# nv-dvl/nerfmatch

Hardware: AMD Instinct MI355X
Metric: rays*samples/sec (higher is better)
Workload: dtype fp16x3 (fp16 MFMA on hi/lo-split fp32 operands, three products per fp32 product, fp32 accumulate; fp32 everywhere else)

## Files before the change

### nerfmatch_amd/csrc/nerf_points_bf16.hip

```cpp
#include "nerf_split_chain.h"

namespace {
using namespace nmbf;
using nmsample::HALF_PI_F32, nmsample::frustum, nmsample::ray_consts, nmsample::lift_var, nmsample::ipe_exact, nmsample::view_row_value;

struct PointsArgs {
  const char* blob;
  const float* xi;
  const float* xd;
  const float* g4;
  float* out4;
  float* g_xi0;
  float* g_xi5;
  float* g_xd;
  u32x4* gates;
  int n, ntiles;
  const float* rays;
  const float* z;
  const float* app_row;
  int S, Sa;
  float* feats;
  const float* tap_w;
  const float* tap_g;
  int tap;
// ... 116 lines not shown
          if (ob < 2) gv0 |= bit; else gv1 |= bit;
          pr = NM_FMA(hv, wr4[e], pr);
          pg = NM_FMA(hv, wg4[e], pg);
          pb = NM_FMA(hv, wb4[e], pb);
        }
      }
    cx.gptr[8 * 256] = u32x4{gv0, gv1, 0u, 0u};
    pr = (pr + nm_shfl_xor32(pr)) + sm_small[OFF_MISC + 1];
    pg = (pg + nm_shfl_xor32(pg)) + sm_small[OFF_MISC + 2];
    pb = (pb + nm_shfl_xor32(pb)) + sm_small[OFF_MISC + 3];
    const float sigma_raw = (cx.sig_part + nm_shfl_xor32(cx.sig_part)) + sm_small[OFF_MISC];
    if (hh == 0 && sample < a.n) *reinterpret_cast<f32x4*>(a.out4 + (size_t)sample * 4) = f32x4{pr, pg, pb, sigma_raw};
  }
}

template <bool GATED>
struct UnitWorkB {
  Ctx& cx;
  Unit& out;
  int u;
  u32x4 gw;
  float v8[8];
  float f0, f1;
  __device__ __forceinline__ void prefetch() {}
  __device__ __forceinline__ void operator()(int j) {
    const int ob = u >> 1, m = u & 1;
    if (j < 4) {
      float a0 = cx.hv[ob * 16 + 8 * m + j], a1 = cx.hv[ob * 16 + 8 * m + 4 + j];
      if constexpr (GATED) {
        const unsigned w = gw[u >> 2];
        const int base = 8 * (u & 3);
        const int e0 = j, e1 = 4 + j;
        const int b0 = base + ((e0 & 1) ? 4 + (e0 >> 1) : (e0 >> 1)), b1 = base + ((e1 & 1) ? 4 + (e1 >> 1) : (e1 >> 1));
        a0 = __int_as_float(__float_as_int(a0) & __builtin_amdgcn_sbfe((int)w, b0, 1));
        a1 = __int_as_float(__float_as_int(a1) & __builtin_amdgcn_sbfe((int)w, b1, 1));
      }
      v8[j] = a0; v8[4 + j] = a1;
      pin(v8[j]); pin(v8[4 + j]);
    } else if (!(j & 1)) {
      const int p = (j - 4) >> 1;
      unsigned hp = pack_bf16(v8[2 * p], v8[2 * p + 1]);
      f0 = __uint_as_float(hp << 16);
      f1 = __uint_as_float(hp & 0xffff0000u);
      pin(hp); pin(f0); pin(f1);
      out.h[p] = hp;
    } else {
      const int p = (j - 5) >> 1;
      float r0 = v8[2 * p] - f0, r1 = v8[2 * p + 1] - f1;
      pin(r0); pin(r1);
      unsigned lp = pack_bf16(r0, r1);
      pin(lp);
      out.l[p] = lp;
    }
  }
};
template <bool GATED>
__device__ __forceinline__ UnitWorkB<GATED> unit_work_b(int u, Ctx& cx, Unit& out, const u32x4& gw) {
  return UnitWorkB<GATED>{cx, out, u, gw, {}, 0.f, 0.f};
}
template <bool GATED>
__device__ __forceinline__ void make_unit0_b(Ctx& cx, const u32x4& gw) {
  UnitWorkB<GATED> w = unit_work_b<GATED>(0, cx, cx.xn, gw);
#pragma unroll
  for (int j = 0; j < 12; ++j) w(j);
}
template <int NOB, int NKS, bool GATED>
__device__ __forceinline__ void bwd_product(f32x16 (&acc)[NOB], Ctx& cx, const u32x4& gw) {
#pragma unroll
  for (int ks = 0; ks < NKS; ks += 2) {
    {
      const Unit xc = cx.xn;
      const bf16x8 xh = __builtin_bit_cast(bf16x8, xc.h), xl = __builtin_bit_cast(bf16x8, xc.l);
      if constexpr (NOB == 8) {
        if (ks == 0) slot_step8<0, true, true>(acc, cx, xh, xl, unit_work_b<GATED>(ks + 1, cx, cx.xn, gw));
        else slot_step8<0, false, true>(acc, cx, xh, xl, unit_work_b<GATED>(ks + 1, cx, cx.xn, gw));
      } else {
        if (ks == 0) slot_step4<0, true, true>(acc, cx, xh, xl, unit_work_b<GATED>(ks + 1, cx, cx.xn, gw));
        else slot_step4<0, false, true>(acc, cx, xh, xl, unit_work_b<GATED>(ks + 1, cx, cx.xn, gw));
      }
    }
    {
      const Unit xc = cx.xn;
      const bf16x8 xh = __builtin_bit_cast(bf16x8, xc.h), xl = __builtin_bit_cast(bf16x8, xc.l);
      if constexpr (NOB == 8) {
        if (ks + 2 < NKS) slot_step8<0, false, false>(acc, cx, xh, xl, unit_work_b<GATED>(ks + 2, cx, cx.xn, gw));
        else slot_step8<0, false, false>(acc, cx, xh, xl, NoWork{});
      } else {
// ... 169 lines not shown
```

### nerfmatch_amd/csrc/nerf_split_chain.h

```cpp
#pragma once
#include "nerf_bf16_common.h"

namespace nmbf {

template <int P> constexpr bool is_bf16() { return P == 0 || P == 4; }
template <int P> constexpr bool has_gates() { return P == 4; }
typedef _Float16 f16x8 __attribute__((ext_vector_type(8)));
typedef _Float16 f16x2 __attribute__((ext_vector_type(2)));
template <int P>
__device__ __forceinline__ f32x16 mfma_p(const bf16x8& a, const bf16x8& b, const f32x16& c) {
  if constexpr (is_bf16<P>()) return MFMA_BF16(a, b, c);
  else return __builtin_amdgcn_mfma_f32_32x32x16_f16(__builtin_bit_cast(f16x8, a), __builtin_bit_cast(f16x8, b), c, 0, 0, 0);
}
template <int P> constexpr bool is_split() { return P != 1; }
template <int P> constexpr int slot_bytes() { return is_split<P>() ? SLOT_BYTES : SLOT_BYTES / 2; }
template <int P> constexpr int slot_floats() { return slot_bytes<P>() / 4; }
template <int P> constexpr int ring_slots() { return is_split<P>() ? NRING : 2 * NRING; }
template <int P> constexpr int ring_ahead() { return is_split<P>() ? 4 : 6; }
constexpr float F16_MAX = 65504.0f;
__device__ __forceinline__ void split8_f16(const float (&v)[8], bf16x8& hi, bf16x8& lo) {
  f16x8 h8, l8;
#pragma unroll
  for (int i = 0; i < 8; ++i) {
    const float c = __builtin_amdgcn_fmed3f(v[i], -F16_MAX, F16_MAX);
// ... 92 lines not shown
      d.l[o] = __builtin_bit_cast(bf16x8, s4[((4 * p + o) * 2 + 1) * 64]);
    } else {
      d.h[o] = __builtin_bit_cast(bf16x8, s4[(4 * p + o) * 64]);
    }
  }
}

struct Ctx {
  const char* blob_slots;
  float* ring;
  const float* sm_small;
  f32x4* tapw;
  bool tap_pref;
  bool rgb;
  float* tap_ring;
  float* tap_ipe;
  int nslots, wave, lane, hi;
  int tap;
  int g;
  unsigned dma_voff;
  unsigned dma_lds;
  OpHalf opA;
  OpHalf opB;
  Unit xn;
  float sig_part;
  float sc;
  float vmax;
  unsigned* rng;
  u32x4* gptr;
  unsigned gbits[4];
  float hv[128];
};

template <int P>
__device__ __forceinline__ void ring_request(const Ctx& cx, int g, int j) {
  const int slot = g + 2 + (j >> 2);
  const char* base = cx.blob_slots + (size_t)slot * slot_bytes<P>();
  const unsigned lds = cx.dma_lds + (unsigned)(slot & (ring_slots<P>() - 1)) * slot_bytes<P>();
  unsigned m0_saved;
#define NM_DMA_PIECE(OFS)                                                                                                        \
  asm volatile("s_mov_b32 %0, m0\n\ts_mov_b32 m0, %1\n\tglobal_load_lds_dwordx4 %2, %3 offset:" #OFS "\n\ts_mov_b32 m0, %0" \
               : "=&s"(m0_saved) : "s"(lds), "v"(cx.dma_voff), "s"(base) : "memory")
  switch (j & 3) {
    case 0: NM_DMA_PIECE(0); break;
    case 1: NM_DMA_PIECE(1024); break;
    case 2: NM_DMA_PIECE(2048); break;
// ... 7 lines not shown
  for (int g0 = 0; g0 < (is_split<P>() ? 2 : ring_ahead<P>()); ++g0) dma_slot<P>(blob_slots, g0, ring, wave, lane);
}
template <int P>
__device__ __forceinline__ void ring_open_wait(Ctx& cx) {
  cx.dma_voff = (unsigned)(cx.wave * (slot_bytes<P>() / 4) + cx.lane * 16);
  const float* q = cx.ring + cx.wave * (slot_floats<P>() / 4);
  cx.dma_lds = (unsigned)__builtin_amdgcn_readfirstlane((int)(unsigned)(size_t)(const __attribute__((address_space(3))) float*)q);
  NM_WAIT_VMCNT(0);
  __builtin_amdgcn_s_barrier();
}

__device__ __forceinline__ unsigned gate_byte(const u32x4& h) {
  const unsigned w0 = h[0], w1 = h[1], w2 = h[2], w3 = h[3];
  unsigned m0, m1, m2, m3;
  const unsigned one = 0x00010001u;
  asm("v_pk_min_u16 %0, %1, %2" : "=v"(m0) : "v"(w0), "v"(one));
  asm("v_pk_min_u16 %0, %1, %2" : "=v"(m1) : "v"(w1), "v"(one));
  asm("v_pk_min_u16 %0, %1, %2" : "=v"(m2) : "v"(w2), "v"(one));
  asm("v_pk_min_u16 %0, %1, %2" : "=v"(m3) : "v"(w3), "v"(one));
  const unsigned t = m0 | (m1 << 1) | (m2 << 2) | (m3 << 3);
  return (t & 0xfu) | ((t >> 12) & 0xf0u);
}

template <int P>
struct UnitWork {
  Ctx& cx;
  Unit& out;
  int u, lo;
  float floor_v;
  f32x4 b0, b1;
  float sc;
  float v8[8];
  float f0, f1;
  unsigned hpk;
  __device__ __forceinline__ void prefetch() {
    const int ob = u >> 1, m = u & 1;
    const float* bl = cx.sm_small + OFF_BIAS + lo * 256 + ob * 32 + 16 * m + 4 * cx.hi;
    b0 = *reinterpret_cast<const f32x4*>(bl); b1 = *reinterpret_cast<const f32x4*>(bl + 8);
  }
  __device__ __forceinline__ void operator()(int j) {
    const int ob = u >> 1, m = u & 1;
    if (j < 4) {
      if constexpr (is_bf16<P>()) {
        v8[j] = __builtin_fmaxf(cx.hv[ob * 16 + 8 * m + j] + b0[j], floor_v);
        v8[4 + j] = __builtin_fmaxf(cx.hv[ob * 16 + 8 * m + 4 + j] + b1[j], floor_v);
      } else if constexpr (P == 1) {
        v8[j] = __builtin_amdgcn_fmed3f(cx.hv[ob * 16 + 8 * m + j] + b0[j], floor_v, F16_MAX);
        v8[4 + j] = __builtin_amdgcn_fmed3f(cx.hv[ob * 16 + 8 * m + 4 + j] + b1[j], floor_v, F16_MAX);
      } else {
        v8[j] = __builtin_amdgcn_fmed3f(__builtin_fmaf(cx.hv[ob * 16 + 8 * m + j], sc, b0[j]), floor_v, F16_MAX);
        v8[4 + j] = __builtin_amdgcn_fmed3f(__builtin_fmaf(cx.hv[ob * 16 + 8 * m + 4 + j], sc, b1[j]), floor_v, F16_MAX);
        asm("v_max3_f32 %0, |%1|, |%2|, %0" : "+v"(cx.vmax) : "v"(v8[j]), "v"(v8[4 + j]));
      }
      pin(v8[j]); pin(v8[4 + j]);
    } else if constexpr (P == 1) {
      if (j < 8) {
        unsigned hp = pack_f16(v8[2 * (j - 4)], v8[2 * (j - 4) + 1]);
        pin(hp);
        out.h[j - 4] = hp;
      }
    } else if (!(j & 1)) {
      const int p = (j - 4) >> 1;
      unsigned hp;
      if constexpr (is_bf16<P>()) {
        hp = pack_bf16(v8[2 * p], v8[2 * p + 1]);
        f0 = __uint_as_float(hp << 16);
        f1 = __uint_as_float(hp & 0xffff0000u);
      } else {
        hp = pack_f16(v8[2 * p], v8[2 * p + 1]);
        hpk = hp;
      }
      pin(hp);
      if constexpr (is_bf16<P>()) { pin(f0); pin(f1); }
      out.h[p] = hp;
    } else {
      const int p = (j - 5) >> 1;
      float r0, r1;
      if constexpr (is_bf16<P>()) {
        r0 = v8[2 * p] - f0; r1 = v8[2 * p + 1] - f1;
      } else {
        asm("v_fma_mix_f32 %0, %1, -1.0, %2 op_sel:[0,0,0] op_sel_hi:[1,0,0]" : "=v"(r0) : "v"(hpk), "v"(v8[2 * p]));
        asm("v_fma_mix_f32 %0, %1, -1.0, %2 op_sel:[1,0,0] op_sel_hi:[1,0,0]" : "=v"(r1) : "v"(hpk), "v"(v8[2 * p + 1]));
      }
      pin(r0); pin(r1);
      unsigned lp = is_bf16<P>() ? pack_bf16(r0, r1) : pack_f16(r0, r1);
      pin(lp);
      out.l[p] = lp;
      if constexpr (has_gates<P>()) {
        if (j == 11) {
          const unsigned t = gate_byte(out.h);
          cx.gbits[u >> 2] |= t << (8 * (u & 3));
        }
      }
    }
  }
};
template <int P>
__device__ __forceinline__ void fold_range(Ctx& cx, int slot) {
  if constexpr (P == 2) {
    const unsigned addr = (unsigned)(size_t)(const __attribute__((address_space(3))) unsigned*)(cx.rng + slot * 256);
    asm volatile("ds_max_u32 %0, %1" :: "v"(addr), "v"(__float_as_uint(cx.vmax)) : "memory");
    cx.vmax = 0.f;
  }
}
struct NoWork {
  __device__ __forceinline__ void prefetch() {}
  __device__ __forceinline__ void operator()(int) {}
};
template <int P>
struct AccTake {
  const f32x16 (&acc)[8];
  Ctx& cx;
  __device__ __forceinline__ void prefetch() {}
  __device__ __forceinline__ void operator()(int j) {
    constexpr int per = is_split<P>() ? 6 : 8;
#pragma unroll
    for (int k = 0; k < per; ++k) {
      const int i = per * j + k;
      if (i < 64) cx.hv[i] = acc_read(acc[i >> 4][i & 15]);
    }
  }
};
template <int P>
__device__ __forceinline__ UnitWork<P> unit_work(int u, int lo, Ctx& cx, Unit& out) {
  return UnitWork<P>{cx, out, u, lo, lo < 8 ? 0.f : (!is_bf16<P>() ? -F16_MAX : -__builtin_inff()), {}, {}, cx.sc, {}, 0.f, 0.f, 0u};
}

template <int P>
__device__ __forceinline__ void finish_layer(const f32x16 (&acc)[8], int l, Ctx& cx) {
#pragma unroll
  for (int ob = 4; ob < 8; ++ob)
#pragma unroll
    for (int r = 0; r < 16; ++r) cx.hv[ob * 16 + r] = acc_read(acc[ob][r]);
  if constexpr (P == 2)
    cx.sc = __builtin_bit_cast(float, __builtin_amdgcn_readfirstlane(__builtin_bit_cast(int, cx.sm_small[OFF_SCALE + l])));
  UnitWork<P> w = unit_work<P>(0, l, cx, cx.xn);
  w.prefetch();
#pragma unroll
  for (int j = 0; j < 12; ++j) w(j);
}

__device__ __forceinline__ void alpha_head(Ctx& cx) {
  const float* bl = cx.sm_small + OFF_BIAS + 7 * 256 + 4 * cx.hi;
  const float* wa = cx.sm_small + OFF_WALPHA + 4 * cx.hi;
  const float s7 = cx.sm_small[OFF_SCALE + 7];
  float p0 = 0.f, p1 = 0.f, p2 = 0.f, p3 = 0.f;
#pragma unroll
  for (int ob = 0; ob < 8; ++ob)
#pragma unroll
    for (int q = 0; q < 4; ++q) {
      const f32x4 b = *reinterpret_cast<const f32x4*>(bl + ob * 32 + 8 * q);
      const f32x4 w4v = *reinterpret_cast<const f32x4*>(wa + ob * 32 + 8 * q);
      p0 = NM_FMA(__builtin_fmaxf(__builtin_fmaf(cx.hv[ob * 16 + 4 * q + 0], s7, b[0]), 0.f), w4v[0], p0);
      p1 = NM_FMA(__builtin_fmaxf(__builtin_fmaf(cx.hv[ob * 16 + 4 * q + 1], s7, b[1]), 0.f), w4v[1], p1);
      p2 = NM_FMA(__builtin_fmaxf(__builtin_fmaf(cx.hv[ob * 16 + 4 * q + 2], s7, b[2]), 0.f), w4v[2], p2);
      p3 = NM_FMA(__builtin_fmaxf(__builtin_fmaf(cx.hv[ob * 16 + 4 * q + 3], s7, b[3]), 0.f), w4v[3], p3);
    }
  cx.sig_part = (p0 + p1) + (p2 + p3);
}

__device__ __forceinline__ void dump_tap(int lo, Ctx& cx) {
  const float* bl = cx.sm_small + OFF_BIAS + lo * 256 + 4 * cx.hi;
  const float sl = cx.sm_small[OFF_SCALE + lo];
  auto* tp = (__attribute__((address_space(1))) f32x4*)cx.tapw;
#pragma unroll
  for (int ob = 0; ob < 8; ++ob) {
    f32x4 v[4];
#pragma unroll
    for (int q = 0; q < 4; ++q) {
      const f32x4 b = *reinterpret_cast<const f32x4*>(bl + ob * 32 + 8 * q);
#pragma unroll
      for (int e = 0; e < 4; ++e) v[q][e] = __builtin_fmaxf(__builtin_fmaf(cx.hv[ob * 16 + 4 * q + e], sl, b[e]), 0.f);
    }
#pragma unroll
    for (int q = 0; q < 4; ++q) tp[q * 64] = v[q];
    tp += 256;
    pin(tp);
  }
}

template <int P, bool FIRST, int NOB>
__device__ __forceinline__ void mfma_head(f32x16 (&acc)[NOB], int p, const OpHalf& a, const bf16x8& xh) {
  const f32x16 zero = {0.f, 0.f, 0.f, 0.f, 0.f, 0.f, 0.f, 0.f, 0.f, 0.f, 0.f, 0.f, 0.f, 0.f, 0.f, 0.f};
#pragma unroll
  for (int o = 0; o < 4; ++o) acc[4 * p + o] = mfma_p<P>(a.h[o], xh, FIRST ? zero : acc[4 * p + o]);
}
template <int P, int NOB>
__device__ __forceinline__ void mfma_tail(f32x16 (&acc)[NOB], int p, const OpHalf& a, const bf16x8& xh, const bf16x8& xl) {
#pragma unroll
  for (int o = 0; o < 4; ++o) acc[4 * p + o] = mfma_p<P>(a.h[o], xl, acc[4 * p + o]);
#pragma unroll
  for (int o = 0; o < 4; ++o) acc[4 * p + o] = mfma_p<P>(a.l[o], xh, acc[4 * p + o]);
}

__device__ __forceinline__ bf16x8 load_op1(const float* slot, int lane, int blk) {
  return __builtin_bit_cast(bf16x8, (reinterpret_cast<const u32x4*>(slot) + lane)[blk * 64]);
}
#define NM_SB __builtin_amdgcn_sched_barrier(0)
template <bool FIRST, bool ACQ, class Work>
__device__ __forceinline__ void slot_step8_one(f32x16 (&acc)[8], Ctx& cx, const bf16x8& x, Work work) {
  const f32x16 zero = {0.f, 0.f, 0.f, 0.f, 0.f, 0.f, 0.f, 0.f, 0.f, 0.f, 0.f, 0.f, 0.f, 0.f, 0.f, 0.f};
  const int g = cx.g;
  const OpHalf A = cx.opA, B = cx.opB;
  const float* nxt = ring_slot<1>(cx.ring, g + 1);
  acc[0] = mfma_p<1>(A.h[0], x, FIRST ? zero : acc[0]); NM_SB;
  if constexpr (ACQ) ring_acquire_pair(cx.blob_slots, g, cx.ring, cx.wave, cx.lane);
  NM_SB;
  acc[1] = mfma_p<1>(A.h[1], x, FIRST ? zero : acc[1]); NM_SB;
  cx.opA.h[0] = load_op1(nxt, cx.lane, 0); cx.opA.h[1] = load_op1(nxt, cx.lane, 1); work.prefetch(); NM_SB;
  acc[2] = mfma_p<1>(A.h[2], x, FIRST ? zero : acc[2]); NM_SB;
  cx.opA.h[2] = load_op1(nxt, cx.lane, 2); cx.opA.h[3] = load_op1(nxt, cx.lane, 3); NM_SB;
  acc[3] = mfma_p<1>(A.h[3], x, FIRST ? zero : acc[3]); NM_SB;
  cx.opB.h[0] = load_op1(nxt, cx.lane, 4); cx.opB.h[1] = load_op1(nxt, cx.lane, 5); NM_SB;
  acc[4] = mfma_p<1>(B.h[0], x, FIRST ? zero : acc[4]); NM_SB;
  cx.opB.h[2] = load_op1(nxt, cx.lane, 6); cx.opB.h[3] = load_op1(nxt, cx.lane, 7); NM_SB;
  acc[5] = mfma_p<1>(B.h[1], x, FIRST ? zero : acc[5]); NM_SB;
  work(0); work(1); NM_SB;
  acc[6] = mfma_p<1>(B.h[2], x, FIRST ? zero : acc[6]); NM_SB;
  work(2); work(3); work(4); NM_SB;
  acc[7] = mfma_p<1>(B.h[3], x, FIRST ? zero : acc[7]); NM_SB;
  work(5); work(6); work(7); NM_SB;
  cx.g = g + 1;
}

template <int P, bool FIRST, bool EVEN, class Work>
__device__ __forceinline__ void slot_step8(f32x16 (&acc)[8], Ctx& cx, const bf16x8& xh, const bf16x8& xl, Work work) {
  if constexpr (P == 1) {
    slot_step8_one<FIRST, EVEN>(acc, cx, xh, work);
    return;
  }
  const f32x16 zero = {0.f, 0.f, 0.f, 0.f, 0.f, 0.f, 0.f, 0.f, 0.f, 0.f, 0.f, 0.f, 0.f, 0.f, 0.f, 0.f};
  const int g = cx.g;
  OpHalf B;
  mfma_head<P, FIRST, 8>(acc, 0, cx.opA, xh);
  __builtin_amdgcn_sched_barrier(0);
  load_half<P>(B, cx.ring + (g & (NRING - 1)) * SLOT_FLOATS, cx.lane, 1);
  work.prefetch();
  __builtin_amdgcn_sched_barrier(0);
  if constexpr (EVEN) {
#pragma unroll
    for (int o = 0; o < 8; ++o) {
      acc[o & 3] = mfma_p<P>(o < 4 ? cx.opA.h[o & 3] : cx.opA.l[o & 3], o < 4 ? xl : xh, acc[o & 3]);
      ring_request<P>(cx, g, o);
      __builtin_amdgcn_sched_barrier(0);
    }
  } else {
    mfma_tail<P, 8>(acc, 0, cx.opA, xh, xl);
    __builtin_amdgcn_sched_barrier(0);
    ring_acquire_two();
    __builtin_amdgcn_sched_barrier(0);
  }
#pragma unroll
  for (int o = 0; o < 4; ++o) {
    acc[4 + o] = mfma_p<P>(B.h[o], xh, FIRST ? zero : acc[4 + o]);
    __builtin_amdgcn_sched_barrier(0);
    work(o);
    __builtin_amdgcn_sched_barrier(0);
  }
  load_half<P>(cx.opA, cx.ring + ((g + 1) & (NRING - 1)) * SLOT_FLOATS, cx.lane, 0);
  __builtin_amdgcn_sched_barrier(0);
#pragma unroll
  for (int o = 0; o < 4; ++o) {
    acc[4 + o] = mfma_p<P>(B.h[o], xl, acc[4 + o]);
    __builtin_amdgcn_sched_barrier(0);
    work(4 + o);
    __builtin_amdgcn_sched_barrier(0);
  }
#pragma unroll
  for (int o = 0; o < 4; ++o) {
    acc[4 + o] = mfma_p<P>(B.l[o], xh, acc[4 + o]);
    __builtin_amdgcn_sched_barrier(0);
    work(8 + o);
    __builtin_amdgcn_sched_barrier(0);
  }
  cx.g = g + 1;
}

template <bool FIRST, bool ACQ, class Work>
__device__ __forceinline__ void slot_step4_one(f32x16 (&acc)[4], Ctx& cx, const bf16x8& x, Work work) {
  const f32x16 zero = {0.f, 0.f, 0.f, 0.f, 0.f, 0.f, 0.f, 0.f, 0.f, 0.f, 0.f, 0.f, 0.f, 0.f, 0.f, 0.f};
  const int g = cx.g;
  const OpHalf C = cx.opA;
  const float* nxt = ring_slot<1>(cx.ring, g + 1);
  acc[0] = mfma_p<1>(C.h[0], x, FIRST ? zero : acc[0]); NM_SB;
  if constexpr (ACQ) ring_acquire_pair(cx.blob_slots, g, cx.ring, cx.wave, cx.lane);
  NM_SB;
  acc[1] = mfma_p<1>(C.h[1], x, FIRST ? zero : acc[1]); NM_SB;
#pragma unroll
  for (int o = 0; o < 4; ++o) cx.opA.h[o] = load_op1(nxt, cx.lane, o);
  work.prefetch(); NM_SB;
  acc[2] = mfma_p<1>(C.h[2], x, FIRST ? zero : acc[2]); NM_SB;
  work(0); work(1); work(2); work(3); NM_SB;
  acc[3] = mfma_p<1>(C.h[3], x, FIRST ? zero : acc[3]); NM_SB;
  work(4); work(5); work(6); work(7); NM_SB;
  cx.g = g + 1;
}

template <int P, bool FIRST, bool EVEN, class Work>
__device__ __forceinline__ void slot_step4(f32x16 (&acc)[4], Ctx& cx, const bf16x8& xh, const bf16x8& xl, Work work) {
  if constexpr (P == 1) {
    slot_step4_one<FIRST, EVEN>(acc, cx, xh, work);
    return;
  }
  const f32x16 zero = {0.f, 0.f, 0.f, 0.f, 0.f, 0.f, 0.f, 0.f, 0.f, 0.f, 0.f, 0.f, 0.f, 0.f, 0.f, 0.f};
  const int g = cx.g;
  const OpHalf C = cx.opA;
  work.prefetch();
  if constexpr (!EVEN) ring_acquire_two();
#pragma unroll
  for (int o = 0; o < 4; ++o) {
    acc[o] = mfma_p<P>(C.h[o], xh, FIRST ? zero : acc[o]);
    __builtin_amdgcn_sched_barrier(0);
    work(o);
    __builtin_amdgcn_sched_barrier(0);
  }
  load_half<P>(cx.opA, cx.ring + ((g + 1) & (NRING - 1)) * SLOT_FLOATS, cx.lane, 0);
  __builtin_amdgcn_sched_barrier(0);
#pragma unroll
  for (int o = 0; o < 4; ++o) {
    acc[o] = mfma_p<P>(C.h[o], xl, acc[o]);
    __builtin_amdgcn_sched_barrier(0);
    if constexpr (EVEN) ring_request<P>(cx, g, o);
    work(4 + o);
    __builtin_amdgcn_sched_barrier(0);
  }
#pragma unroll
  for (int o = 0; o < 4; ++o) {
    acc[o] = mfma_p<P>(C.l[o], xh, acc[o]);
    __builtin_amdgcn_sched_barrier(0);
    if constexpr (EVEN) ring_request<P>(cx, g, 4 + o);
    work(8 + o);
    __builtin_amdgcn_sched_barrier(0);
  }
  cx.g = g + 1;
}

template <int P, bool FIRST, bool EVEN, class W0, class W1>
__device__ __forceinline__ void slot_step4x2(f32x16 (&av)[4], Ctx& cx, const bf16x8& x0h, const bf16x8& x0l, Unit& u1, W0 w0, W1 w1) {
  const f32x16 zero = {0.f, 0.f, 0.f, 0.f, 0.f, 0.f, 0.f, 0.f, 0.f, 0.f, 0.f, 0.f, 0.f, 0.f, 0.f, 0.f};
  const int g = cx.g;
  const OpHalf A = cx.opA;
  OpHalf B;
  w0.prefetch();
#pragma unroll
  for (int o = 0; o < 4; ++o) {
    av[o] = mfma_p<P>(A.h[o], x0h, FIRST ? zero : av[o]);
    __builtin_amdgcn_sched_barrier(0);
    w0(o);
    __builtin_amdgcn_sched_barrier(0);
  }
  load_half<P>(B, cx.ring + (g & (NRING - 1)) * SLOT_FLOATS, cx.lane, 1);
  __builtin_amdgcn_sched_barrier(0);
#pragma unroll
  for (int o = 0; o < 4; ++o) {
    av[o] = mfma_p<P>(A.h[o], x0l, av[o]);
    __builtin_amdgcn_sched_barrier(0);
    if constexpr (EVEN) ring_request<P>(cx, g, o);
    w0(4 + o);
    __builtin_amdgcn_sched_barrier(0);
  }
#pragma unroll
  for (int o = 0; o < 4; ++o) {
    av[o] = mfma_p<P>(A.l[o], x0h, av[o]);
    __builtin_amdgcn_sched_barrier(0);
    if constexpr (EVEN) ring_request<P>(cx, g, 4 + o);
    w0(8 + o);
    __builtin_amdgcn_sched_barrier(0);
  }
  if constexpr (!EVEN) {
    ring_acquire_two();
    __builtin_amdgcn_sched_barrier(0);
  }
  const bf16x8 x1h = __builtin_bit_cast(bf16x8, u1.h), x1l = __builtin_bit_cast(bf16x8, u1.l);
  w1.prefetch();
#pragma unroll
  for (int o = 0; o < 4; ++o) {
    av[o] = mfma_p<P>(B.h[o], x1h, av[o]);
    __builtin_amdgcn_sched_barrier(0);
    w1(o);
    __builtin_amdgcn_sched_barrier(0);
  }
  load_half<P>(cx.opA, cx.ring + ((g + 1) & (NRING - 1)) * SLOT_FLOATS, cx.lane, 0);
  __builtin_amdgcn_sched_barrier(0);
#pragma unroll
  for (int o = 0; o < 4; ++o) {
    av[o] = mfma_p<P>(B.h[o], x1l, av[o]);
    __builtin_amdgcn_sched_barrier(0);
    w1(4 + o);
    __builtin_amdgcn_sched_barrier(0);
  }
#pragma unroll
  for (int o = 0; o < 4; ++o) {
    av[o] = mfma_p<P>(B.l[o], x1h, av[o]);
    __builtin_amdgcn_sched_barrier(0);
    w1(8 + o);
    __builtin_amdgcn_sched_barrier(0);
  }
  cx.g = g + 1;
}

template <int P>
__device__ __forceinline__ void views_hidden(f32x16 (&av)[4], Ctx& cx) {
  if constexpr (is_split<P>()) {
#pragma unroll
    for (int sl = 0; sl < HS / 2; ++sl) {
      const Unit x0 = cx.xn;
      Unit u1;
      const bf16x8 x0h = __builtin_bit_cast(bf16x8, x0.h), x0l = __builtin_bit_cast(bf16x8, x0.l);
      if (sl == 0) slot_step4x2<P, true, true>(av, cx, x0h, x0l, u1, unit_work<P>(1, 7, cx, u1), unit_work<P>(2, 7, cx, cx.xn));
      else if (sl + 1 == HS / 2) slot_step4x2<P, false, false>(av, cx, x0h, x0l, u1, unit_work<P>(2 * sl + 1, 7, cx, u1), NoWork{});
      else if (sl & 1) slot_step4x2<P, false, false>(av, cx, x0h, x0l, u1, unit_work<P>(2 * sl + 1, 7, cx, u1), unit_work<P>(2 * sl + 2, 7, cx, cx.xn));
      else slot_step4x2<P, false, true>(av, cx, x0h, x0l, u1, unit_work<P>(2 * sl + 1, 7, cx, u1), unit_work<P>(2 * sl + 2, 7, cx, cx.xn));
    }
  } else {
#pragma unroll
    for (int ks = 0; ks < HS; ks += 2) {
      {
        const Unit xc = cx.xn;
// ... 3 lines not shown
      {
        const Unit xc = cx.xn;
        if (ks + 2 < HS) slot_step4<P, false, false>(av, cx, __builtin_bit_cast(bf16x8, xc.h), __builtin_bit_cast(bf16x8, xc.l), unit_work<P>(ks + 2, 7, cx, cx.xn));
        else slot_step4<P, false, false>(av, cx, __builtin_bit_cast(bf16x8, xc.h), __builtin_bit_cast(bf16x8, xc.l), NoWork{});
      }
    }
  }
}
template <int P>
__device__ __forceinline__ void views_extras(f32x16 (&av)[4], Ctx& cx, const bf16x8 (&eh)[VS], const bf16x8 (&el)[VS], bool no_app) {
  if constexpr (is_split<P>()) {
    Unit u1;
    u1.h = __builtin_bit_cast(u32x4, eh[1]); u1.l = __builtin_bit_cast(u32x4, el[1]);
    slot_step4x2<P, false, true>(av, cx, eh[0], el[0], u1, NoWork{}, NoWork{});
    if (!no_app) slot_step4<P, false, false>(av, cx, eh[2], el[2], NoWork{});
  } else {
    slot_step4<P, false, true>(av, cx, eh[0], el[0], NoWork{});
    slot_step4<P, false, false>(av, cx, eh[1], el[1], NoWork{});
    if (!no_app) slot_step4<P, false, true>(av, cx, eh[2], el[2], NoWork{});
  }
}

template <int P, bool FIRST>
__device__ __forceinline__ void ipe_steps(f32x16 (&acc)[8], Ctx& cx, const float* ipe_src) {
  auto operand = [&](int m, bf16x8& ph, bf16x8& pl) {
    ph = __builtin_bit_cast(bf16x8, *reinterpret_cast<const u32x4*>(ipe_src + (is_split<P>() ? (m * 2 + 0) : m) * 256));
    pl = ph;
    if constexpr (is_split<P>()) pl = __builtin_bit_cast(bf16x8, *reinterpret_cast<const u32x4*>(ipe_src + (m * 2 + 1) * 256));
  };
#pragma unroll
  for (int m = 0; m < XS; m += 2) {
    bf16x8 ph, pl;
    operand(m, ph, pl);
    if (m == 0) slot_step8<P, FIRST, true>(acc, cx, ph, pl, NoWork{});
    else slot_step8<P, false, true>(acc, cx, ph, pl, NoWork{});
    operand(m + 1, ph, pl);
    if (m + 2 == XS) slot_step8<P, false, false>(acc, cx, ph, pl, AccTake<P>{acc, cx});
    else slot_step8<P, false, false>(acc, cx, ph, pl, NoWork{});
  }
}

struct Tap7Workspace {
  static constexpr bool on = false;
  __device__ __forceinline__ void fn(Ctx&) const {}
};
template <class F>
struct Tap7InRegisters {
  bool on;
  F fn;
};

template <int P, class Tap7 = Tap7Workspace>
__device__ __forceinline__ void layer_pass(f32x16 (&acc)[8], int l, Ctx& cx, const float* ipe_src, const Tap7& tap7 = Tap7()) {
  if (l - 1 == cx.tap) dump_tap(l - 1, cx);
#pragma unroll
  for (int ks = 0; ks < HS; ks += 2) {
    {
      const Unit xc = cx.xn;
      if (ks == 0) slot_step8<P, true, true>(acc, cx, __builtin_bit_cast(bf16x8, xc.h), __builtin_bit_cast(bf16x8, xc.l), unit_work<P>(ks + 1, l - 1, cx, cx.xn));
      else slot_step8<P, false, true>(acc, cx, __builtin_bit_cast(bf16x8, xc.h), __builtin_bit_cast(bf16x8, xc.l), unit_work<P>(ks + 1, l - 1, cx, cx.xn));
    }
    {
      const Unit xc = cx.xn;
      if (ks + 2 < HS) slot_step8<P, false, false>(acc, cx, __builtin_bit_cast(bf16x8, xc.h), __builtin_bit_cast(bf16x8, xc.l), unit_work<P>(ks + 2, l - 1, cx, cx.xn));
      else slot_step8<P, false, false>(acc, cx, __builtin_bit_cast(bf16x8, xc.h), __builtin_bit_cast(bf16x8, xc.l), AccTake<P>{acc, cx});
    }
  }
  fold_range<P>(cx, l - 1);
  if constexpr (has_gates<P>()) {
    cx.gptr[(l - 1) * 256] = u32x4{cx.gbits[0], cx.gbits[1], cx.gbits[2], cx.gbits[3]};
    cx.gbits[0] = cx.gbits[1] = cx.gbits[2] = cx.gbits[3] = 0u;
  }
  if (l == 5) ipe_steps<P, false>(acc, cx, ipe_src);
  finish_layer<P>(acc, l, cx);
  if (l == 7) {
    if (cx.rgb) {
      if (cx.tap == 7 && !tap7.on) dump_tap(7, cx);
      alpha_head(cx);
      if (tap7.on) tap7.fn(cx);
    }
  }
}

}
```

Baseline: 359.2 million.

## Reschedule split-MFMA slot steps with interleaved operand loads and staged unit work

Rewrites the slot_step8/4/4x2 inner loops as a single 12-MFMA loop per operand half. Operand loads for the next slot are split into per-output pairs spread across MFMA slots instead of issued as one block. Unit activation/packing work is broken into fine-grained stages (bias, relu halves, hi, remainder, lo, gates) placed by explicit per-slot schedules. Accumulator draining (AccTake) is also spread across slots, with the next layer's bias prefetched into Ctx. The aim is to hide VALU and LDS latency under MFMA issue, at the cost of more live registers and a fragile hand-tuned schedule.

```diff
diff --git a/nerfmatch_amd/csrc/nerf_points_bf16.hip b/nerfmatch_amd/csrc/nerf_points_bf16.hip
--- a/nerfmatch_amd/csrc/nerf_points_bf16.hip
+++ b/nerfmatch_amd/csrc/nerf_points_bf16.hip
@@ -162,47 +162,52 @@
   u32x4 gw;
   float v8[8];
   float f0, f1;
-  __device__ __forceinline__ void prefetch() {}
-  __device__ __forceinline__ void operator()(int j) {
-    const int ob = u >> 1, m = u & 1;
-    if (j < 4) {
-      float a0 = cx.hv[ob * 16 + 8 * m + j], a1 = cx.hv[ob * 16 + 8 * m + 4 + j];
-      if constexpr (GATED) {
-        const unsigned w = gw[u >> 2];
-        const int base = 8 * (u & 3);
-        const int e0 = j, e1 = 4 + j;
-        const int b0 = base + ((e0 & 1) ? 4 + (e0 >> 1) : (e0 >> 1)), b1 = base + ((e1 & 1) ? 4 + (e1 >> 1) : (e1 >> 1));
-        a0 = __int_as_float(__float_as_int(a0) & __builtin_amdgcn_sbfe((int)w, b0, 1));
-        a1 = __int_as_float(__float_as_int(a1) & __builtin_amdgcn_sbfe((int)w, b1, 1));
-      }
-      v8[j] = a0; v8[4 + j] = a1;
-      pin(v8[j]); pin(v8[4 + j]);
-    } else if (!(j & 1)) {
-      const int p = (j - 4) >> 1;
-      unsigned hp = pack_bf16(v8[2 * p], v8[2 * p + 1]);
-      f0 = __uint_as_float(hp << 16);
-      f1 = __uint_as_float(hp & 0xffff0000u);
-      pin(hp); pin(f0); pin(f1);
-      out.h[p] = hp;
-    } else {
-      const int p = (j - 5) >> 1;
-      float r0 = v8[2 * p] - f0, r1 = v8[2 * p + 1] - f1;
-      pin(r0); pin(r1);
-      unsigned lp = pack_bf16(r0, r1);
-      pin(lp);
-      out.l[p] = lp;
-    }
-  }
+  float r0[4], r1[4];
+  __device__ __forceinline__ float gated(int e) const {
+    float a = cx.hv[(u >> 1) * 16 + 8 * (u & 1) + e];
+    if constexpr (GATED) {
+      const int b = 8 * (u & 3) + ((e & 1) ? 4 + (e >> 1) : (e >> 1));
+      a = __int_as_float(__float_as_int(a) & __builtin_amdgcn_sbfe((int)gw[u >> 2], b, 1));
+    }
+    return a;
+  }
+  __device__ __forceinline__ void bias() {}
+  __device__ __forceinline__ void ra(int j) { v8[j] = gated(j); pin(v8[j]); }
+  __device__ __forceinline__ void rb(int j) { v8[4 + j] = gated(4 + j); pin(v8[4 + j]); }
+  __device__ __forceinline__ void relu(int j) { ra(j); rb(j); }
+  __device__ __forceinline__ void hi(int p) {
+    unsigned hp = pack_bf16(v8[2 * p], v8[2 * p + 1]);
+    f0 = __uint_as_float(hp << 16);
+    f1 = __uint_as_float(hp & 0xffff0000u);
+    pin(hp); pin(f0); pin(f1);
+    out.h[p] = hp;
+  }
+  __device__ __forceinline__ void rem(int p) {
+    r0[p] = v8[2 * p] - f0; r1[p] = v8[2 * p + 1] - f1;
+    pin(r0[p]); pin(r1[p]);
+  }
+  __device__ __forceinline__ void lo(int p) {
+    unsigned lp = pack_bf16(r0[p], r1[p]);
+    pin(lp);
+    out.l[p] = lp;
+  }
+  __device__ __forceinline__ void gates() {}
+  __device__ __forceinline__ void seq(int c) { unit_seq<true>(*this, c); }
+  template <bool EVEN> __device__ __forceinline__ void step8(int t) { unit_step8<EVEN, true>(*this, t); }
 };
 template <bool GATED>
 __device__ __forceinline__ UnitWorkB<GATED> unit_work_b(int u, Ctx& cx, Unit& out, const u32x4& gw) {
-  return UnitWorkB<GATED>{cx, out, u, gw, {}, 0.f, 0.f};
+  return UnitWorkB<GATED>{cx, out, u, gw, {}, 0.f, 0.f, {}, {}};
 }
 template <bool GATED>
 __device__ __forceinline__ void make_unit0_b(Ctx& cx, const u32x4& gw) {
   UnitWorkB<GATED> w = unit_work_b<GATED>(0, cx, cx.xn, gw);
 #pragma unroll
-  for (int j = 0; j < 12; ++j) w(j);
+  for (int j = 0; j < 4; ++j) w.relu(j);
+#pragma unroll
+  for (int p = 0; p < 4; ++p) { w.hi(p); w.rem(p); }
+#pragma unroll
+  for (int p = 0; p < 4; ++p) w.lo(p);
 }
 template <int NOB, int NKS, bool GATED>
 __device__ __forceinline__ void bwd_product(f32x16 (&acc)[NOB], Ctx& cx, const u32x4& gw) {
diff --git a/nerfmatch_amd/csrc/nerf_split_chain.h b/nerfmatch_amd/csrc/nerf_split_chain.h
--- a/nerfmatch_amd/csrc/nerf_split_chain.h
+++ b/nerfmatch_amd/csrc/nerf_split_chain.h
@@ -138,6 +138,7 @@
   unsigned dma_lds;
   OpHalf opA;
   OpHalf opB;
+  f32x4 hb0, hb1;
   Unit xn;
   float sig_part;
   float sc;
@@ -191,79 +192,132 @@
   return (t & 0xfu) | ((t >> 12) & 0xf0u);
 }
 
+template <bool BF, class W> __device__ __forceinline__ void unit_seq(W& w, int c);
+template <bool EVEN, bool BF, class W> __device__ __forceinline__ void unit_step8(W& w, int t);
 template <int P>
 struct UnitWork {
   Ctx& cx;
   Unit& out;
-  int u, lo;
+  int u, lo_;
   float floor_v;
   f32x4 b0, b1;
   float sc;
   float v8[8];
   float f0, f1;
-  unsigned hpk;
-  __device__ __forceinline__ void prefetch() {
+  float r0[4], r1[4];
+  __device__ __forceinline__ void bias() {
     const int ob = u >> 1, m = u & 1;
-    const float* bl = cx.sm_small + OFF_BIAS + lo * 256 + ob * 32 + 16 * m + 4 * cx.hi;
+    const float* bl = cx.sm_small + OFF_BIAS + lo_ * 256 + ob * 32 + 16 * m + 4 * cx.hi;
     b0 = *reinterpret_cast<const f32x4*>(bl); b1 = *reinterpret_cast<const f32x4*>(bl + 8);
   }
+  __device__ __forceinline__ float act(int e, float b) const {
+    const float h = cx.hv[(u >> 1) * 16 + 8 * (u & 1) + e];
+    if constexpr (is_bf16<P>()) return __builtin_fmaxf(h + b, floor_v);
+    else if constexpr (P == 1) return __builtin_amdgcn_fmed3f(h + b, floor_v, F16_MAX);
+    else return __builtin_amdgcn_fmed3f(__builtin_fmaf(h, sc, b), floor_v, F16_MAX);
+  }
+  __device__ __forceinline__ void range(int j) {
+    if constexpr (P == 2) asm("v_max3_f32 %0, |%1|, |%2|, %0" : "+v"(cx.vmax) : "v"(v8[j]), "v"(v8[4 + j]));
+  }
+  __device__ __forceinline__ void ra(int j) { v8[j] = act(j, b0[j]); pin(v8[j]); }
+  __device__ __forceinline__ void rb(int j) { v8[4 + j] = act(4 + j, b1[j]); range(j); pin(v8[4 + j]); }
+  __device__ __forceinline__ void relu(int j) {
+    v8[j] = act(j, b0[j]); v8[4 + j] = act(4 + j, b1[j]);
+    range(j);
+    pin(v8[j]); pin(v8[4 + j]);
+  }
+  __device__ __forceinline__ void hi(int p) {
+    unsigned hp;
+    if constexpr (is_bf16<P>()) {
+      hp = pack_bf16(v8[2 * p], v8[2 * p + 1]);
+      f0 = __uint_as_float(hp << 16);
+      f1 = __uint_as_float(hp & 0xffff0000u);
+    } else {
+      hp = pack_f16(v8[2 * p], v8[2 * p + 1]);
+    }
+    pin(hp);
+    if constexpr (is_bf16<P>()) { pin(f0); pin(f1); }
+    out.h[p] = hp;
+  }
+  __device__ __forceinline__ void rem(int p) {
+    if constexpr (is_bf16<P>()) {
+      r0[p] = v8[2 * p] - f0; r1[p] = v8[2 * p + 1] - f1;
+      pin(r0[p]); pin(r1[p]);
+    } else {
+      asm volatile("v_fma_mix_f32 %0, %1, -1.0, %2 op_sel:[0,0,0] op_sel_hi:[1,0,0]" : "=v"(r0[p]) : "v"(out.h[p]), "v"(v8[2 * p]));
+      asm volatile("v_fma_mix_f32 %0, %1, -1.0, %2 op_sel:[1,0,0] op_sel_hi:[1,0,0]" : "=v"(r1[p]) : "v"(out.h[p]), "v"(v8[2 * p + 1]));
+    }
+  }
+  __device__ __forceinline__ void lo(int p) {
+    unsigned lp = is_bf16<P>() ? pack_bf16(r0[p], r1[p]) : pack_f16(r0[p], r1[p]);
+    pin(lp);
+    out.l[p] = lp;
+  }
+  __device__ __forceinline__ void gates() {
+    if constexpr (has_gates<P>()) {
+      const unsigned t = gate_byte(out.h);
+      cx.gbits[u >> 2] |= t << (8 * (u & 3));
+    }
+  }
+  __device__ __forceinline__ void seq(int c) { unit_seq<is_bf16<P>()>(*this, c); }
+  template <bool EVEN> __device__ __forceinline__ void step8(int t) { unit_step8<EVEN, is_bf16<P>()>(*this, t); }
+  __device__ __forceinline__ void prefetch() { bias(); }
   __device__ __forceinline__ void operator()(int j) {
-    const int ob = u >> 1, m = u & 1;
-    if (j < 4) {
-      if constexpr (is_bf16<P>()) {
-        v8[j] = __builtin_fmaxf(cx.hv[ob * 16 + 8 * m + j] + b0[j], floor_v);
-        v8[4 + j] = __builtin_fmaxf(cx.hv[ob * 16 + 8 * m + 4 + j] + b1[j], floor_v);
-      } else if constexpr (P == 1) {
-        v8[j] = __builtin_amdgcn_fmed3f(cx.hv[ob * 16 + 8 * m + j] + b0[j], floor_v, F16_MAX);
-        v8[4 + j] = __builtin_amdgcn_fmed3f(cx.hv[ob * 16 + 8 * m + 4 + j] + b1[j], floor_v, F16_MAX);
-      } else {
-        v8[j] = __builtin_amdgcn_fmed3f(__builtin_fmaf(cx.hv[ob * 16 + 8 * m + j], sc, b0[j]), floor_v, F16_MAX);
-        v8[4 + j] = __builtin_amdgcn_fmed3f(__builtin_fmaf(cx.hv[ob * 16 + 8 * m + 4 + j], sc, b1[j]), floor_v, F16_MAX);
-        asm("v_max3_f32 %0, |%1|, |%2|, %0" : "+v"(cx.vmax) : "v"(v8[j]), "v"(v8[4 + j]));
-      }
-      pin(v8[j]); pin(v8[4 + j]);
-    } else if constexpr (P == 1) {
+    if (j < 4) relu(j);
+    else if constexpr (P == 1) {
       if (j < 8) {
         unsigned hp = pack_f16(v8[2 * (j - 4)], v8[2 * (j - 4) + 1]);
         pin(hp);
         out.h[j - 4] = hp;
       }
-    } else if (!(j & 1)) {
-      const int p = (j - 4) >> 1;
-      unsigned hp;
-      if constexpr (is_bf16<P>()) {
-        hp = pack_bf16(v8[2 * p], v8[2 * p + 1]);
-        f0 = __uint_as_float(hp << 16);
-        f1 = __uint_as_float(hp & 0xffff0000u);
-      } else {
-        hp = pack_f16(v8[2 * p], v8[2 * p + 1]);
-        hpk = hp;
-      }
-      pin(hp);
-      if constexpr (is_bf16<P>()) { pin(f0); pin(f1); }
-      out.h[p] = hp;
-    } else {
-      const int p = (j - 5) >> 1;
-      float r0, r1;
-      if constexpr (is_bf16<P>()) {
-        r0 = v8[2 * p] - f0; r1 = v8[2 * p + 1] - f1;
-      } else {
-        asm("v_fma_mix_f32 %0, %1, -1.0, %2 op_sel:[0,0,0] op_sel_hi:[1,0,0]" : "=v"(r0) : "v"(hpk), "v"(v8[2 * p]));
-        asm("v_fma_mix_f32 %0, %1, -1.0, %2 op_sel:[1,0,0] op_sel_hi:[1,0,0]" : "=v"(r1) : "v"(hpk), "v"(v8[2 * p + 1]));
-      }
-      pin(r0); pin(r1);
-      unsigned lp = is_bf16<P>() ? pack_bf16(r0, r1) : pack_f16(r0, r1);
-      pin(lp);
-      out.l[p] = lp;
-      if constexpr (has_gates<P>()) {
-        if (j == 11) {
-          const unsigned t = gate_byte(out.h);
-          cx.gbits[u >> 2] |= t << (8 * (u & 3));
-        }
-      }
+    } else if (!(j & 1)) hi((j - 4) >> 1);
+    else {
+      rem((j - 5) >> 1); lo((j - 5) >> 1);
+      if (j == 11) gates();
     }
   }
 };
+template <bool BF, class W>
+__device__ __forceinline__ void unit_seq(W& w, int c) {
+  switch (c) {
+    case 0: w.bias(); break;
+    case 2: w.ra(0); break;
+    case 3: w.rb(0); break;
+    case 4: w.ra(1); break;
+    case 5: w.rb(1); w.ra(2); break;
+    case 6: w.rb(2); w.ra(3); break;
+    case 7: w.rb(3); w.hi(0); break;
+    case 8: if constexpr (BF) { w.rem(0); w.hi(1); } else { w.hi(1); w.hi(2); w.hi(3); w.rem(0); } break;
+    case 9: if constexpr (BF) { w.rem(1); w.hi(2); } else { w.lo(0); w.rem(1); w.rem(2); } break;
+    case 10: if constexpr (BF) { w.rem(2); w.hi(3); } else { w.lo(1); w.lo(2); w.rem(3); } break;
+    case 11: if constexpr (BF) { w.rem(3); w.lo(0); w.lo(1); w.lo(2); w.lo(3); w.gates(); } else { w.lo(3); } break;
+    default: break;
+  }
+}
+template <bool EVEN, bool BF, class W>
+__device__ __forceinline__ void unit_step8(W& w, int t) {
+  if constexpr (EVEN) {
+    if (t >= 12) unit_seq<BF>(w, t - 12);
+  } else {
+    switch (t) {
+      case 4: w.bias(); break;
+      case 6: case 7: case 8: case 9: w.relu(t - 6); break;
+      case 10: if constexpr (BF) { w.hi(0); } else { w.hi(0); w.hi(1); w.hi(2); w.hi(3); } break;
+      case 11: if constexpr (BF) { w.rem(0); } else { w.rem(0); w.rem(1); } break;
+      case 12: if constexpr (BF) { w.hi(1); } else { w.lo(0); w.lo(1); w.rem(2); } break;
+      case 13: w.rem(BF ? 1 : 3); break;
+      case 14: if constexpr (BF) { w.lo(0); w.lo(1); } else { w.lo(2); } break;
+      case 15: if constexpr (!BF) { w.lo(3); } break;
+      case 17: if constexpr (BF) { w.hi(2); } break;
+      case 18: if constexpr (BF) { w.rem(2); } break;
+      case 19: if constexpr (BF) { w.hi(3); w.lo(2); } break;
+      case 20: if constexpr (BF) { w.rem(3); } break;
+      case 21: if constexpr (BF) { w.lo(3); } break;
+      case 22: if constexpr (BF) { w.gates(); } break;
+      default: break;
+    }
+  }
+}
 template <int P>
 __device__ __forceinline__ void fold_range(Ctx& cx, int slot) {
   if constexpr (P == 2) {
@@ -275,28 +329,56 @@
 struct NoWork {
   __device__ __forceinline__ void prefetch() {}
   __device__ __forceinline__ void operator()(int) {}
+  __device__ __forceinline__ void seq(int) {}
+  template <bool EVEN> __device__ __forceinline__ void step8(int) {}
 };
+constexpr int take_n(int s) { return s == 0 ? 4 : s == 1 ? 2 : s <= 4 ? 3 : s == 10 ? 2 : 5; }
+constexpr int take_before(int s) {
+  int n = 0;
+  for (int k = 0; k < s; ++k) n += take_n(k);
+  return n;
+}
+constexpr int TAKE_HIDDEN = take_before(12);
+__device__ __forceinline__ const float* unit0_bias(const Ctx& cx, int l) { return cx.sm_small + OFF_BIAS + l * 256 + 4 * cx.hi; }
 template <int P>
 struct AccTake {
   const f32x16 (&acc)[8];
   Ctx& cx;
+  int l;
   __device__ __forceinline__ void prefetch() {}
   __device__ __forceinline__ void operator()(int j) {
-    constexpr int per = is_split<P>() ? 6 : 8;
-#pragma unroll
-    for (int k = 0; k < per; ++k) {
-      const int i = per * j + k;
+#pragma unroll
+    for (int k = 0; k < 8; ++k) {
+      const int i = 8 * j + k;
       if (i < 64) cx.hv[i] = acc_read(acc[i >> 4][i & 15]);
     }
   }
+  __device__ __forceinline__ void seq(int) {}
+  template <bool EVEN> __device__ __forceinline__ void step8(int t) {
+    if (t < 12) return;
+    const int s = t - 12;
+#pragma unroll
+    for (int k = 0; k < take_n(s); ++k) {
+      const int i = take_before(s) + k;
+      cx.hv[i] = acc_read(acc[i >> 4][i & 15]);
+    }
+    if (s == 10) {
+      const float* bl = unit0_bias(cx, l);
+      cx.hb0 = *reinterpret_cast<const f32x4*>(bl); cx.hb1 = *reinterpret_cast<const f32x4*>(bl + 8);
+    }
+  }
 };
 template <int P>
 __device__ __forceinline__ UnitWork<P> unit_work(int u, int lo, Ctx& cx, Unit& out) {
-  return UnitWork<P>{cx, out, u, lo, lo < 8 ? 0.f : (!is_bf16<P>() ? -F16_MAX : -__builtin_inff()), {}, {}, cx.sc, {}, 0.f, 0.f, 0u};
+  return UnitWork<P>{cx, out, u, lo, lo < 8 ? 0.f : (!is_bf16<P>() ? -F16_MAX : -__builtin_inff()), {}, {}, cx.sc, {}, 0.f, 0.f, {}, {}};
 }
 
 template <int P>
 __device__ __forceinline__ void finish_layer(const f32x16 (&acc)[8], int l, Ctx& cx) {
+  if constexpr (is_split<P>()) {
+#pragma unroll
+    for (int i = TAKE_HIDDEN; i < 64; ++i) cx.hv[i] = acc_read(acc[i >> 4][i & 15]);
+  }
 #pragma unroll
   for (int ob = 4; ob < 8; ++ob)
 #pragma unroll
@@ -304,9 +386,27 @@
   if constexpr (P == 2)
     cx.sc = __builtin_bit_cast(float, __builtin_amdgcn_readfirstlane(__builtin_bit_cast(int, cx.sm_small[OFF_SCALE + l])));
   UnitWork<P> w = unit_work<P>(0, l, cx, cx.xn);
-  w.prefetch();
-#pragma unroll
-  for (int j = 0; j < 12; ++j) w(j);
+  if constexpr (is_split<P>()) {
+    w.b0 = cx.hb0; w.b1 = cx.hb1;
+#pragma unroll
+    for (int j = 0; j < 4; ++j) w.relu(j);
+#pragma unroll
+    for (int p = 0; p < 4; ++p) {
+      w.hi(p);
+      if constexpr (is_bf16<P>()) w.rem(p);
+    }
+    if constexpr (!is_bf16<P>()) {
+#pragma unroll
+      for (int p = 0; p < 4; ++p) w.rem(p);
+    }
+#pragma unroll
+    for (int p = 0; p < 4; ++p) w.lo(p);
+    w.gates();
+  } else {
+    w.prefetch();
+#pragma unroll
+    for (int j = 0; j < 12; ++j) w(j);
+  }
 }
 
 __device__ __forceinline__ void alpha_head(Ctx& cx) {
@@ -346,20 +446,6 @@
     tp += 256;
     pin(tp);
   }
-}
-
-template <int P, bool FIRST, int NOB>
-__device__ __forceinline__ void mfma_head(f32x16 (&acc)[NOB], int p, const OpHalf& a, const bf16x8& xh) {
-  const f32x16 zero = {0.f, 0.f, 0.f, 0.f, 0.f, 0.f, 0.f, 0.f, 0.f, 0.f, 0.f, 0.f, 0.f, 0.f, 0.f, 0.f};
-#pragma unroll
-  for (int o = 0; o < 4; ++o) acc[4 * p + o] = mfma_p<P>(a.h[o], xh, FIRST ? zero : acc[4 * p + o]);
-}
-template <int P, int NOB>
-__device__ __forceinline__ void mfma_tail(f32x16 (&acc)[NOB], int p, const OpHalf& a, const bf16x8& xh, const bf16x8& xl) {
-#pragma unroll
-  for (int o = 0; o < 4; ++o) acc[4 * p + o] = mfma_p<P>(a.h[o], xl, acc[4 * p + o]);
-#pragma unroll
-  for (int o = 0; o < 4; ++o) acc[4 * p + o] = mfma_p<P>(a.l[o], xh, acc[4 * p + o]);
 }
 
 __device__ __forceinline__ bf16x8 load_op1(const float* slot, int lane, int blk) {
@@ -392,54 +478,52 @@
   cx.g = g + 1;
 }
 
+template <int P>
+__device__ __forceinline__ void load_pair(OpHalf& d, const float* slot, int lane, int p, int o) {
+  const u32x4* s4 = reinterpret_cast<const u32x4*>(slot) + lane;
+  d.h[o] = __builtin_bit_cast(bf16x8, s4[((4 * p + o) * 2 + 0) * 64]);
+  d.l[o] = __builtin_bit_cast(bf16x8, s4[((4 * p + o) * 2 + 1) * 64]);
+}
+template <int P, bool FIRST>
+__device__ __forceinline__ f32x16 mfma_k(int k, const OpHalf& a, const bf16x8& xh, const bf16x8& xl, const f32x16& c) {
+  const f32x16 zero = {0.f, 0.f, 0.f, 0.f, 0.f, 0.f, 0.f, 0.f, 0.f, 0.f, 0.f, 0.f, 0.f, 0.f, 0.f, 0.f};
+  if (k < 4) return mfma_p<P>(a.h[k], xh, FIRST ? zero : c);
+  if (k < 8) return mfma_p<P>(a.h[k & 3], xl, c);
+  return mfma_p<P>(a.l[k & 3], xh, c);
+}
+
 template <int P, bool FIRST, bool EVEN, class Work>
 __device__ __forceinline__ void slot_step8(f32x16 (&acc)[8], Ctx& cx, const bf16x8& xh, const bf16x8& xl, Work work) {
   if constexpr (P == 1) {
     slot_step8_one<FIRST, EVEN>(acc, cx, xh, work);
     return;
   }
-  const f32x16 zero = {0.f, 0.f, 0.f, 0.f, 0.f, 0.f, 0.f, 0.f, 0.f, 0.f, 0.f, 0.f, 0.f, 0.f, 0.f, 0.f};
   const int g = cx.g;
+  const OpHalf A = cx.opA;
   OpHalf B;
-  mfma_head<P, FIRST, 8>(acc, 0, cx.opA, xh);
-  __builtin_amdgcn_sched_barrier(0);
-  load_half<P>(B, cx.ring + (g & (NRING - 1)) * SLOT_FLOATS, cx.lane, 1);
-  work.prefetch();
-  __builtin_amdgcn_sched_barrier(0);
-  if constexpr (EVEN) {
-#pragma unroll
-    for (int o = 0; o < 8; ++o) {
-      acc[o & 3] = mfma_p<P>(o < 4 ? cx.opA.h[o & 3] : cx.opA.l[o & 3], o < 4 ? xl : xh, acc[o & 3]);
-      ring_request<P>(cx, g, o);
-      __builtin_amdgcn_sched_barrier(0);
-    }
-  } else {
-    mfma_tail<P, 8>(acc, 0, cx.opA, xh, xl);
-    __builtin_amdgcn_sched_barrier(0);
+  const float* cur = cx.ring + (g & (NRING - 1)) * SLOT_FLOATS;
+  const float* nxt = cx.ring + ((g + 1) & (NRING - 1)) * SLOT_FLOATS;
+#pragma unroll
+  for (int k = 0; k < 12; ++k) {
+    acc[k & 3] = mfma_k<P, FIRST>(k, A, xh, xl, acc[k & 3]);
+    __builtin_amdgcn_sched_barrier(0);
+    if (k < 4) load_pair<P>(B, cur, cx.lane, 1, k);
+    if constexpr (EVEN) {
+      if (k >= 4) ring_request<P>(cx, g, k - 4);
+    }
+    work.template step8<EVEN>(k);
+    __builtin_amdgcn_sched_barrier(0);
+  }
+  if constexpr (!EVEN) {
     ring_acquire_two();
     __builtin_amdgcn_sched_barrier(0);
   }
 #pragma unroll
-  for (int o = 0; o < 4; ++o) {
-    acc[4 + o] = mfma_p<P>(B.h[o], xh, FIRST ? zero : acc[4 + o]);
-    __builtin_amdgcn_sched_barrier(0);
-    work(o);
-    __builtin_amdgcn_sched_barrier(0);
-  }
-  load_half<P>(cx.opA, cx.ring + ((g + 1) & (NRING - 1)) * SLOT_FLOATS, cx.lane, 0);
-  __builtin_amdgcn_sched_barrier(0);
-#pragma unroll
-  for (int o = 0; o < 4; ++o) {
-    acc[4 + o] = mfma_p<P>(B.h[o], xl, acc[4 + o]);
-    __builtin_amdgcn_sched_barrier(0);
-    work(4 + o);
-    __builtin_amdgcn_sched_barrier(0);
-  }
-#pragma unroll
-  for (int o = 0; o < 4; ++o) {
-    acc[4 + o] = mfma_p<P>(B.l[o], xh, acc[4 + o]);
-    __builtin_amdgcn_sched_barrier(0);
-    work(8 + o);
+  for (int k = 0; k < 12; ++k) {
+    acc[4 + (k & 3)] = mfma_k<P, FIRST>(k, B, xh, xl, acc[4 + (k & 3)]);
+    __builtin_amdgcn_sched_barrier(0);
+    if (k >= 1 && k <= 4) load_pair<P>(cx.opA, nxt, cx.lane, 0, k - 1);
+    work.template step8<EVEN>(12 + k);
     __builtin_amdgcn_sched_barrier(0);
   }
   cx.g = g + 1;
@@ -471,34 +555,19 @@
     slot_step4_one<FIRST, EVEN>(acc, cx, xh, work);
     return;
   }
-  const f32x16 zero = {0.f, 0.f, 0.f, 0.f, 0.f, 0.f, 0.f, 0.f, 0.f, 0.f, 0.f, 0.f, 0.f, 0.f, 0.f, 0.f};
   const int g = cx.g;
   const OpHalf C = cx.opA;
-  work.prefetch();
+  const float* nxt = cx.ring + ((g + 1) & (NRING - 1)) * SLOT_FLOATS;
   if constexpr (!EVEN) ring_acquire_two();
 #pragma unroll
-  for (int o = 0; o < 4; ++o) {
-    acc[o] = mfma_p<P>(C.h[o], xh, FIRST ? zero : acc[o]);
-    __builtin_amdgcn_sched_barrier(0);
-    work(o);
-    __builtin_amdgcn_sched_barrier(0);
-  }
-  load_half<P>(cx.opA, cx.ring + ((g + 1) & (NRING - 1)) * SLOT_FLOATS, cx.lane, 0);
-  __builtin_amdgcn_sched_barrier(0);
-#pragma unroll
-  for (int o = 0; o < 4; ++o) {
-    acc[o] = mfma_p<P>(C.h[o], xl, acc[o]);
-    __builtin_amdgcn_sched_barrier(0);
-    if constexpr (EVEN) ring_request<P>(cx, g, o);
-    work(4 + o);
-    __builtin_amdgcn_sched_barrier(0);
-  }
-#pragma unroll
-  for (int o = 0; o < 4; ++o) {
-    acc[o] = mfma_p<P>(C.l[o], xh, acc[o]);
-    __builtin_amdgcn_sched_barrier(0);
-    if constexpr (EVEN) ring_request<P>(cx, g, 4 + o);
-    work(8 + o);
+  for (int k = 0; k < 12; ++k) {
+    acc[k & 3] = mfma_k<P, FIRST>(k, C, xh, xl, acc[k & 3]);
+    __builtin_amdgcn_sched_barrier(0);
+    if (k >= 1 && k <= 4) load_pair<P>(cx.opA, nxt, cx.lane, 0, k - 1);
+    if constexpr (EVEN) {
+      if (k >= 4) ring_request<P>(cx, g, k - 4);
+    }
+    work.seq(k);
     __builtin_amdgcn_sched_barrier(0);
   }
   cx.g = g + 1;
@@ -506,34 +575,20 @@
 
 template <int P, bool FIRST, bool EVEN, class W0, class W1>
 __device__ __forceinline__ void slot_step4x2(f32x16 (&av)[4], Ctx& cx, const bf16x8& x0h, const bf16x8& x0l, Unit& u1, W0 w0, W1 w1) {
-  const f32x16 zero = {0.f, 0.f, 0.f, 0.f, 0.f, 0.f, 0.f, 0.f, 0.f, 0.f, 0.f, 0.f, 0.f, 0.f, 0.f, 0.f};
   const int g = cx.g;
   const OpHalf A = cx.opA;
   OpHalf B;
-  w0.prefetch();
-#pragma unroll
-  for (int o = 0; o < 4; ++o) {
-    av[o] = mfma_p<P>(A.h[o], x0h, FIRST ? zero : av[o]);
-    __builtin_amdgcn_sched_barrier(0);
-    w0(o);
-    __builtin_amdgcn_sched_barrier(0);
-  }
-  load_half<P>(B, cx.ring + (g & (NRING - 1)) * SLOT_FLOATS, cx.lane, 1);
-  __builtin_amdgcn_sched_barrier(0);
-#pragma unroll
-  for (int o = 0; o < 4; ++o) {
-    av[o] = mfma_p<P>(A.h[o], x0l, av[o]);
-    __builtin_amdgcn_sched_barrier(0);
-    if constexpr (EVEN) ring_request<P>(cx, g, o);
-    w0(4 + o);
-    __builtin_amdgcn_sched_barrier(0);
-  }
-#pragma unroll
-  for (int o = 0; o < 4; ++o) {
-    av[o] = mfma_p<P>(A.l[o], x0h, av[o]);
-    __builtin_amdgcn_sched_barrier(0);
-    if constexpr (EVEN) ring_request<P>(cx, g, 4 + o);
-    w0(8 + o);
+  const float* cur = cx.ring + (g & (NRING - 1)) * SLOT_FLOATS;
+  const float* nxt = cx.ring + ((g + 1) & (NRING - 1)) * SLOT_FLOATS;
+#pragma unroll
+  for (int k = 0; k < 12; ++k) {
+    av[k & 3] = mfma_k<P, FIRST>(k, A, x0h, x0l, av[k & 3]);
+    __builtin_amdgcn_sched_barrier(0);
+    if (k >= 1 && k <= 4) load_pair<P>(B, cur, cx.lane, 1, k - 1);
+    if constexpr (EVEN) {
+      if (k >= 4) ring_request<P>(cx, g, k - 4);
+    }
+    w0.seq(k);
     __builtin_amdgcn_sched_barrier(0);
   }
   if constexpr (!EVEN) {
@@ -541,28 +596,12 @@
     __builtin_amdgcn_sched_barrier(0);
   }
   const bf16x8 x1h = __builtin_bit_cast(bf16x8, u1.h), x1l = __builtin_bit_cast(bf16x8, u1.l);
-  w1.prefetch();
-#pragma unroll
-  for (int o = 0; o < 4; ++o) {
-    av[o] = mfma_p<P>(B.h[o], x1h, av[o]);
-    __builtin_amdgcn_sched_barrier(0);
-    w1(o);
-    __builtin_amdgcn_sched_barrier(0);
-  }
-  load_half<P>(cx.opA, cx.ring + ((g + 1) & (NRING - 1)) * SLOT_FLOATS, cx.lane, 0);
-  __builtin_amdgcn_sched_barrier(0);
-#pragma unroll
-  for (int o = 0; o < 4; ++o) {
-    av[o] = mfma_p<P>(B.h[o], x1l, av[o]);
-    __builtin_amdgcn_sched_barrier(0);
-    w1(4 + o);
-    __builtin_amdgcn_sched_barrier(0);
-  }
-#pragma unroll
-  for (int o = 0; o < 4; ++o) {
-    av[o] = mfma_p<P>(B.l[o], x1h, av[o]);
-    __builtin_amdgcn_sched_barrier(0);
-    w1(8 + o);
+#pragma unroll
+  for (int k = 0; k < 12; ++k) {
+    av[k & 3] = mfma_k<P, false>(k, B, x1h, x1l, av[k & 3]);
+    __builtin_amdgcn_sched_barrier(0);
+    if (k >= 1 && k <= 4) load_pair<P>(cx.opA, nxt, cx.lane, 0, k - 1);
+    w1.seq(k);
     __builtin_amdgcn_sched_barrier(0);
   }
   cx.g = g + 1;
@@ -612,7 +651,7 @@
 }
 
 template <int P, bool FIRST>
-__device__ __forceinline__ void ipe_steps(f32x16 (&acc)[8], Ctx& cx, const float* ipe_src) {
+__device__ __forceinline__ void ipe_steps(f32x16 (&acc)[8], Ctx& cx, const float* ipe_src, int l = FIRST ? 0 : 5) {
   auto operand = [&](int m, bf16x8& ph, bf16x8& pl) {
     ph = __builtin_bit_cast(bf16x8, *reinterpret_cast<const u32x4*>(ipe_src + (is_split<P>() ? (m * 2 + 0) : m) * 256));
     pl = ph;
@@ -625,7 +664,7 @@
     if (m == 0) slot_step8<P, FIRST, true>(acc, cx, ph, pl, NoWork{});
     else slot_step8<P, false, true>(acc, cx, ph, pl, NoWork{});
     operand(m + 1, ph, pl);
-    if (m + 2 == XS) slot_step8<P, false, false>(acc, cx, ph, pl, AccTake<P>{acc, cx});
+    if (m + 2 == XS) slot_step8<P, false, false>(acc, cx, ph, pl, AccTake<P>{acc, cx, l});
     else slot_step8<P, false, false>(acc, cx, ph, pl, NoWork{});
   }
 }
@@ -653,7 +692,7 @@
     {
       const Unit xc = cx.xn;
       if (ks + 2 < HS) slot_step8<P, false, false>(acc, cx, __builtin_bit_cast(bf16x8, xc.h), __builtin_bit_cast(bf16x8, xc.l), unit_work<P>(ks + 2, l - 1, cx, cx.xn));
-      else slot_step8<P, false, false>(acc, cx, __builtin_bit_cast(bf16x8, xc.h), __builtin_bit_cast(bf16x8, xc.l), AccTake<P>{acc, cx});
+      else slot_step8<P, false, false>(acc, cx, __builtin_bit_cast(bf16x8, xc.h), __builtin_bit_cast(bf16x8, xc.l), AccTake<P>{acc, cx, l});
     }
   }
   fold_range<P>(cx, l - 1);
```

Result: faster. 373.3 million (median of 6 runs) (+3.9%).
